# fawnliu/TRIS

Measured on AMD Instinct MI355X. Metric: Stage-1 training images/sec @320px bs48 (TRIS clip-RN50, 3 negatives), higher is better.
Workload: dtype f32 storage/accumulate; products h2 = 2 x f16 pieces; 1 GPU; Stage-1 train step, RefCOCOg-shaped synthetic batch: 48 img/GPU 320x320, 20-token query + 3 negative queries per image, clip-RN50 trunk + frozen aux CLIP ViT-B/32, AdamW (BASELINE.json configs[2]/[3]); per_gpu_batch=48, global_batch=48, size=320, query_len=20, negative_samples=3, parallelism=dp1, sync_bn=False

## Files before the change

### include/tris_hip.h

```cpp
#ifndef TRIS_HIP_H
#define TRIS_HIP_H

#ifdef __cplusplus
extern "C" {
#endif

int tris_gemm_f32(const float* A, const float* B, float* C, int M, int N, int K, long lda, long ldb, long ldc,
                  int transA, int transB, int batch, long strideA, long strideB, long strideC, const float* bias,
                  int bias_mode, const float* resid, long ldr, long strideR, int act, float alpha, float* workspace,
                  long workspace_bytes, void* stream);

int tris_gemm_epilogue_next(float* pre_out, const float* dact_x);

int tris_splitk_tickets_next(int* tickets, int count);
long tris_splitk_fused_launches(void);

int tris_set_gemm_mode(int mode);
int tris_set_gemm_mode_thread(int mode);
int tris_set_option(const char* name, const char* value);
int tris_set_conv_direct_thread(int value);

int tris_set_autotune(int on);
int tris_get_autotune(void);
int tris_get_gemm_mode(void);
// ... 183 lines not shown
int tris_maps_bwd_f32(const float* score, const float* d_relu, const float* d_sig, float* dscore, int B, int h, int w,
                      int N, int S, void* stream);
int tris_resize_bilinear_fwd_f32(const float* X, float* Y, int planes, int Hi, int Wi, int Ho, int Wo,
                                 int align_corners, void* stream);
int tris_resize_bilinear_bwd_f32(const float* dY, float* dX, int planes, int Hi, int Wi, int Ho, int Wo,
                                 int align_corners, void* stream);
int tris_fg_patch_fwd_f32(const float* cam, const float* img, float* patches, int B, int C, int R, int ps,
                          void* stream);
int tris_fg_patch_bwd_f32(const float* dpatches, const float* img, float* dcam, int B, int C, int R, int ps,
                          void* stream);
int tris_vit_assemble_fwd_f32(const float* emb, const float* cls, const float* pos, float* x, int B, int T, int W,
                              void* stream);
int tris_vit_assemble_bwd_f32(const float* dx, float* demb, int B, int T, int W, void* stream);
int tris_stage1_loss_fwd_f32(const float* cls, const float* fi, const float* ft, const float* fneg, int B, int N, int E,
                             int K, float w1, float w4, float w5, float* per_img, float* rowloss, float* losses,
                             void* stream);
int tris_stage1_loss_bwd_f32(const float* cls, const float* fi, const float* ft, const float* fneg, const float* g,
                             float w1, float w4, float w5, int B, int N, int E, int K, float* dcls, float* dfi, void* stream);

int tris_adamw_f32(float* p, const float* g, float* m, float* v, long n, float lr, float beta1, float beta2, float eps,
                   float weight_decay, int step_count, void* stream);
int tris_adamw_dev_f32(float* p, const float* g, float* m, float* v, long n, const float* hyper, float beta1, float beta2,
                       float eps, float weight_decay, void* stream);

int tris_eval_post_f32(const float* relu_map, int S, const unsigned char* target, int oH, int oW, float* cam,
                       long* out_iu, float* workspace , void* stream);

int tris_resample_u8(const unsigned char* in, int Hin, int Win, int C, const int* bounds_h, const int* kk_h, int ksize_h,
                     const int* bounds_v, const int* kk_v, int ksize_v, int Hout, int Wout, unsigned char* tmp,
                     unsigned char* out, void* stream);
int tris_gather2d_u8(const unsigned char* in, int Hin, int Win, int C, const int* yidx, const int* xidx, int Hout,
                     int Wout, unsigned char* out, void* stream);
int tris_mask_sum_nearest_u8(const unsigned char* masks, int K, int Hin, int Win, const int* yidx, const int* xidx,
                             int Hout, int Wout, unsigned char* out, void* stream);
int tris_u8_gather_normalize_f32(const unsigned char* cache, const long* index, int B, long HW, const float* lut,
                                 float* out, int planar, void* stream);
int tris_gather_rows(const void* table, const long* index, long rows, long row_bytes, void* out, void* stream);

#define TRIS_MBOX_MAX_WORLD 16
long tris_mbox_bytes(int cap_floats);
int tris_mbox_alloc(void** ptr, int cap_floats);
int tris_mbox_free(void* ptr);
int tris_mbox_ipc_handle(void* ptr, void* handle64);
int tris_mbox_ipc_open(const void* handle64, void** ptr);
int tris_mbox_ipc_close(void* ptr);
int tris_mbox_exchange_f32(const float* src0, int n0, const float* src1, int n1, float* out, void* const* boxes, int world,
// ... 77 lines not shown
```

### tris_amd/config.py

```python
import contextlib
import os


def _flag(name, default):
    v = os.environ.get(name)
    return default if v is None or v == "" else v != "0"


class _Config:
    def __setattr__(self, name, value):
        if name == "step_graph" and "step_graph" in self.__dict__:
            self.__dict__["step_graph_chosen"] = True
        self.__dict__[name] = value

    def __init__(self):
        e = os.environ.get
        self.step_graph = e("TRIS_STEP_GRAPH", "0")
        self.step_graph_chosen = "TRIS_STEP_GRAPH" in os.environ
        self.hipgraph = _flag("TRIS_HIPGRAPH", True)
        self.text_stream = _flag("TRIS_TEXT_STREAM", True)
        self.wgrad_stream = _flag("TRIS_WGRAD_STREAM", True)
        self.stream_probe = _flag("TRIS_STREAM_PROBE", True)
        self.stream_probe_log = e("TRIS_STREAM_PROBE_LOG") == "1"
        self.text_at = e("TRIS_TEXT_AT", "layer4")
# ... 7 lines not shown
        self.ddp_seg_poison = _flag("TRIS_DDP_SEG_POISON", False)
        self.syncbn_bound = _flag("TRIS_SYNCBN_BOUND", True)
        self.xattn_fused = _flag("TRIS_XATTN_FUSED", True)
        self.xattn_px = _flag("TRIS_XATTN_PX", True)
        self.xattn_h2 = _flag("TRIS_XATTN_H2", True)
        self.xattn_bwd_px = _flag("TRIS_XATTN_BWD_PX", True)
        self.hbm_loader = _flag("TRIS_HBM_LOADER", True)
        self.eval_group = max(1, int(e("TRIS_EVAL_GROUP", "16")))
        self.mbox_spin = int(e("TRIS_MBOX_SPIN", "40000000"))
        self.syncbn_comm = e("TRIS_SYNCBN_COMM", "mailbox")
        self.ddp_check = e("TRIS_DDP_CHECK") == "1"
        self.ddp_sparse_embed = _flag("TRIS_DDP_SPARSE_EMBED", True)
        self.random_init = e("TRIS_RANDOM_INIT") == "1"
        self.h2_planes = _flag("TRIS_H2_PLANES", True)
        self.own_stream = _flag("TRIS_OWN_STREAM", True)
        self.fuse_splitk = _flag("TRIS_FUSE_SPLITK_PY", False)
        self.aux_text_early = _flag("TRIS_AUX_TEXT_EARLY", True)
        self.text_pack = _flag("TRIS_TEXT_PACK", True)
        self.bn_bitmask = _flag("TRIS_BN_BITMASK", True)
        self.gemm_convert = int(e("TRIS_GEMM_CONVERT", "0"))
        self.step_graph_rerecord = int(e("TRIS_STEP_GRAPH_RERECORD", "3"))
        self.side_param_grads = _flag("TRIS_SIDE_PARAM_GRADS", True)
        self.vit_token0 = _flag("TRIS_VIT_TOKEN0", True)

    @contextlib.contextmanager
    def override(self, **kw):
        old = {k: getattr(self, k) for k in kw}
        try:
            for k, v in kw.items():
                setattr(self, k, v)
            yield self
        finally:
            for k, v in old.items():
                setattr(self, k, v)

    def key(self):
        return tuple(sorted((k, v) for k, v in self.__dict__.items() if k not in ("step_graph_chosen", "step_graph_rerecord")))


cfg = _Config()
```

### tris_amd/csrc/optim.hip

```cpp
#include "common.h"
#include "tris_hip.h"

namespace {
__global__ __launch_bounds__(256) void adamw_kernel(float* __restrict__ p, const float* __restrict__ g,
                                                    float* __restrict__ m, float* __restrict__ v, long n, float lr,
                                                    float b1, float b2, float eps, float wd, float bc1, float bc2s) {
  long i = (long)blockIdx.x * blockDim.x + threadIdx.x;
  const long stride = (long)gridDim.x * blockDim.x;
  const long n4 = n >> 2;
  const float decay = 1.0f - lr * wd, step = lr / bc1;
  for (long j = i; j < n4; j += stride) {
    float4 P = *reinterpret_cast<float4*>(p + j * 4), G = *reinterpret_cast<const float4*>(g + j * 4);
    float4 M = *reinterpret_cast<float4*>(m + j * 4), V = *reinterpret_cast<float4*>(v + j * 4);
#define TRIS_ADAM1(e)                       \
  P.e *= decay;                             \
  M.e = b1 * M.e + (1.0f - b1) * G.e;       \
  V.e = b2 * V.e + (1.0f - b2) * G.e * G.e; \
  P.e -= step * M.e / (sqrtf(V.e) / bc2s + eps);
    TRIS_ADAM1(x) TRIS_ADAM1(y) TRIS_ADAM1(z) TRIS_ADAM1(w)
#undef TRIS_ADAM1
    *reinterpret_cast<float4*>(p + j * 4) = P;
    *reinterpret_cast<float4*>(m + j * 4) = M;
    *reinterpret_cast<float4*>(v + j * 4) = V;
  }
  for (long j = n4 * 4 + i; j < n; j += stride) {
    float P = p[j] * decay, G = g[j];
    float M = b1 * m[j] + (1.0f - b1) * G, V = b2 * v[j] + (1.0f - b2) * G * G;
    p[j] = P - step * M / (sqrtf(V) / bc2s + eps);
    m[j] = M;
    v[j] = V;
  }
}
__global__ __launch_bounds__(256) void adamw_dev_kernel(float* __restrict__ p, const float* __restrict__ g,
                                                        float* __restrict__ m, float* __restrict__ v, long n,
                                                        const float* __restrict__ hyper, float b1, float b2, float eps,
                                                        float wd) {
  const float lr = hyper[0], bc1 = hyper[1], bc2s = hyper[2];
  long i = (long)blockIdx.x * blockDim.x + threadIdx.x;
  const long stride = (long)gridDim.x * blockDim.x;
  const long n4 = n >> 2;
  const float decay = 1.0f - lr * wd, step = lr / bc1;
  for (long j = i; j < n4; j += stride) {
    float4 P = *reinterpret_cast<float4*>(p + j * 4), G = *reinterpret_cast<const float4*>(g + j * 4);
    float4 M = *reinterpret_cast<float4*>(m + j * 4), V = *reinterpret_cast<float4*>(v + j * 4);
#define TRIS_ADAM1(e)                       \
  P.e *= decay;                             \
  M.e = b1 * M.e + (1.0f - b1) * G.e;       \
  V.e = b2 * V.e + (1.0f - b2) * G.e * G.e; \
  P.e -= step * M.e / (sqrtf(V.e) / bc2s + eps);
    TRIS_ADAM1(x) TRIS_ADAM1(y) TRIS_ADAM1(z) TRIS_ADAM1(w)
#undef TRIS_ADAM1
    *reinterpret_cast<float4*>(p + j * 4) = P;
    *reinterpret_cast<float4*>(m + j * 4) = M;
    *reinterpret_cast<float4*>(v + j * 4) = V;
  }
  for (long j = n4 * 4 + i; j < n; j += stride) {
    float P = p[j] * decay, G = g[j];
    float M = b1 * m[j] + (1.0f - b1) * G, V = b2 * v[j] + (1.0f - b2) * G * G;
    p[j] = P - step * M / (sqrtf(V) / bc2s + eps);
    m[j] = M;
    v[j] = V;
  }
}
}

extern "C" int tris_adamw_f32(float* p, const float* g, float* m, float* v, long n, float lr, float beta1, float beta2,
                              float eps, float weight_decay, int step_count, void* stream) {
  double bc1 = 1.0 - pow((double)beta1, (double)step_count);
  double bc2 = 1.0 - pow((double)beta2, (double)step_count);
  long g4 = (n / 4 + 255) / 256;
  if (g4 > 8192) g4 = 8192;
  if (g4 < 1) g4 = 1;
  hipLaunchKernelGGL(adamw_kernel, dim3((unsigned)g4), dim3(256), 0, (hipStream_t)stream, p, g, m, v, n, lr, beta1,
                     beta2, eps, weight_decay, (float)bc1, (float)sqrt(bc2));
  TRIS_LAUNCH_CHECK();
  return 0;
}

extern "C" int tris_adamw_dev_f32(float* p, const float* g, float* m, float* v, long n, const float* hyper, float beta1,
                                  float beta2, float eps, float weight_decay, void* stream) {
  long g4 = (n / 4 + 255) / 256;
  if (g4 > 8192) g4 = 8192;
  if (g4 < 1) g4 = 1;
  hipLaunchKernelGGL(adamw_dev_kernel, dim3((unsigned)g4), dim3(256), 0, (hipStream_t)stream, p, g, m, v, n, hyper, beta1,
                     beta2, eps, weight_decay);
  TRIS_LAUNCH_CHECK();
  return 0;
}
```

### tris_amd/graphs.py

```python


import torch


class NotCapturable(RuntimeError):
    """the step cannot be replayed from hipGraphs in this configuration (train_step then runs it eagerly)"""


class GraphedStage1Eval:
    def __init__(self, net, img_shape, query_len, warmup=2):
        assert not net.training, "capture the eval path (model.eval())"
        self.net = net
        dev = next(net.parameters()).device
        self.s_img = torch.zeros(img_shape, device=dev, dtype=torch.float32)
        self.s_ids = torch.zeros(img_shape[0], query_len, device=dev, dtype=torch.int64)
        self.s_ids[:, 0] = 49406
        self.s_ids[:, 1] = 49407
        H = img_shape[2]
        from . import ops
        self.h2_vis, self.h2_txt = ops.h2_private_pool(), ops.h2_private_pool()
        with torch.no_grad():
            side = torch.cuda.Stream()
            side.wait_stream(torch.cuda.current_stream())
            with torch.cuda.stream(side):
# ... 45 lines not shown
        self.s_ids.copy_(ids, non_blocking=True)
        self.g.replay()
        return self.out.clone()


class GraphedTrainStep:

    def __init__(self, model, clip_model, optimizer, args, example, lr_scheduler=None, priming=2):
        from . import ops
        from .CLIP.clip.model import BatchNorm2d
        from .train_stage1 import _step_body
        img, ids, neg = example
        self.model, self.clip_model, self.optimizer, self.args, self.sched = model, clip_model, optimizer, args, lr_scheduler
        self.s_img = img.detach().clone()
        self.s_ids = ids.detach().clone()
        self.s_neg = None if neg is None else neg.detach().clone()
        net = model.module if hasattr(model, "module") else model
        self.bns = [m for m in net.modules() if isinstance(m, BatchNorm2d)]
        optimizer.enable_device_hyper()
        _prime(model, clip_model, optimizer, self.bns, (self.s_img, self.s_ids, self.s_neg), args, priming)
        nbt = [m._nbt_pending for m in self.bns]
        self.g = torch.cuda.CUDAGraph()
        ops._CAPTURE_STREAMS = True
        try:
            with torch.cuda.graph(self.g, capture_error_mode="thread_local"):
                self.losses = _step_body(model, clip_model, optimizer, self.s_img, self.s_ids, self.s_neg, args, None,
                                         device_hyper=True)
        finally:
            ops._CAPTURE_STREAMS = False
        for m, n in zip(self.bns, nbt):
            m._nbt_pending = n

    def __call__(self, img, ids, neg):
        self.s_img.copy_(img, non_blocking=True)
        self.s_ids.copy_(ids, non_blocking=True)
        if self.s_neg is not None:
            self.s_neg.copy_(neg, non_blocking=True)
        opt = self.optimizer
        opt._steps += 1
        opt.push_hyper()
        self.g.replay()
        for m in self.bns:
            m._nbt_pending += 1
        if self.sched is not None:
            self.sched.step()
        return self.losses


def _prime(model, clip_model, optimizer, bns, batch, args, priming, reducer=None):
    from .train_stage1 import _step_body
    keep = [(m.running_mean.clone(), m.running_var.clone(), m._nbt_pending) for m in bns]
    for _ in range(priming):
        _step_body(model, clip_model, optimizer, batch[0], batch[1], batch[2], args, reducer, optimizer_step=False)
    torch.cuda.synchronize()
    with torch.no_grad():
        for m, (rm, rv, nbt) in zip(bns, keep):
            m.running_mean.copy_(rm)
            m.running_var.copy_(rv)
            m._nbt_pending = nbt
    del keep
    torch.cuda.synchronize()
    torch.cuda.empty_cache()


# ... 137 lines not shown
                keys, self.released = self.released, []
                return keys
            g = G()
            _capture(g, self.cap, pool_c, b_heads)
            self.back = [(g,) + wgrad_graphs()[:2] + (take_released(),)]
            self.inline = True
            self.g_btext = G()
            _capture(self.g_btext, self.text, pool_t, lambda: torch.autograd.backward(hidden, h.grad))
            self.inline = False
            self.text_released = take_released()
            n_late = min(6, len(trunk_cuts))
            split = True
            late_sinks = []
            for k, (x, leaf) in enumerate(reversed(trunk_cuts)):
                late = k >= len(trunk_cuts) - n_late
                g = G()
                _capture(g, self.cap, pool_c, lambda: torch.autograd.backward(x, leaf.grad))
                gw, gt, sinks = wgrad_graphs(split=late and split)
                self.back.append((g, gw, gt, take_released()))
                if late:
                    late_sinks += sinks
            self.first_late = len(self.back) - n_late
            spans = self._late_spans(optimizer, late_sinks) if (n_late and self.reducer is None) else None
            self.g_opt_early = None
            if spans:
                early = []
                for gi, a in enumerate(optimizer.arenas):
                    lo, hi = spans.get(gi, (0, 0))
                    early += [(gi, 0, lo), (gi, hi, a.numel)] if hi > lo else [(gi, 0, a.numel)]
                self.g_opt_early = G()
                _capture(self.g_opt_early, self.cap, pool_c, lambda: optimizer.step(device_hyper=True, ranges=early))
                rest = [(gi, lo, hi) for gi, (lo, hi) in spans.items()]
            else:
                rest = None
            self.g_opt_seg, self.g_opt_ranges, self._poisoned, self.poisoned_segments = {}, {}, [], 0
            red = self.reducer
            if red is not None and cfg.ddp_seg_opt and red.segments:
                released = [k for (_, _, _, keys) in self.back for k in keys] + list(self.text_released)
                pool_o = torch.cuda.graph_pool_handle()
                covered = {}
                for k in released:
                    segs = [(ai, s_, e_) for ai, s_, e_ in red.segments.get(k, []) if e_ > s_]
                    if not segs or k in self.g_opt_seg or sorted(red._dense_ranges(k)) != sorted(segs):
                        continue
                    g = G()
                    _capture(g, self.cap, pool_o, lambda: optimizer.step(device_hyper=True, ranges=segs))
                    self.g_opt_seg[k] = g
                    self.g_opt_ranges[k] = segs
                    for ai, s_, e_ in segs:
                        covered.setdefault(ai, []).append((s_, e_))
                if self.g_opt_seg:
                    rest = []
                    for gi, a in enumerate(optimizer.arenas):
                        cur = 0
                        for s_, e_ in sorted(covered.get(gi, [])):
                            if s_ > cur:
                                rest.append((gi, cur, s_))
                            cur = max(cur, e_)
                        if cur < a.numel:
                            rest.append((gi, cur, a.numel))
            self.g_opt = G()
            _capture(self.g_opt, self.cap, pool_c, lambda: optimizer.step(device_hyper=True, ranges=rest))
        finally:
            ops._SEG = None
            ops.h2_end_step()
            self.cuts, self.deferred = [], []
            if gc_was:
                gc.enable()
        del keep, trunk_cuts, h, hidden, vis, late_sinks, fwd
        for m, n in zip(self.bns, nbt):
            m._nbt_pending = n
        self.ev = [torch.cuda.Event() for _ in range(len(self.back) + 8)]
        self.trace = False
        self._marks = None

    def _reduce_and_update(self, red, key):
        from . import ops
        if key in red.done or not red.active:
            return
        n0 = len(red.pending)
        red._launch_now(key)
        g = self.g_opt_seg.get(key)
        if g is not None:
            with torch.cuda.stream(ops.side_stream("reduce")):
                for h in red.pending[n0:]:
# ... 45 lines not shown

    def release(self, key):
        self.released.append(key)

    def defer(self, fn, tensors, sink):
        if self.inline:
            return fn()
        self.deferred.append((fn, tensors, sink))
        return None

    def __call__(self, img, ids, neg):
        from . import ops
        main, text, wg, ev = torch.cuda.current_stream(), self.text, self.wg, self.ev
        tm = self._marks = [] if self.trace else None

        def mark(name, stream=main):
            if tm is not None:
                e = torch.cuda.Event(enable_timing=True)
                e.record(stream)
                tm.append((name, e))
        mark("start")
        if self.h2_pool is not None:
            self.h2_pool.zero_()
            ops.h2_weights_amax(self.h2_arenas)
        self.s_img.copy_(img, non_blocking=True)
        self.s_ids.copy_(ids, non_blocking=True)
        if self.s_neg is not None:
            self.s_neg.copy_(neg, non_blocking=True)
        opt = self.optimizer
        opt._steps += 1
        opt.push_hyper()
        ev[0].record(main)
        fm = self.fwd_marks
        from .config import cfg as _cfg
        aux_early = bool(_cfg.aux_text_early)
        for i, g in enumerate(self.fwd):
            if i == fm.get("text", 0):
                if i:
                    ev[0].record(main)
                text.wait_event(ev[0])
                with torch.cuda.stream(text):
                    self.g_ftext.replay()
                    ev[1].record(text)
                    mark("text_fwd_done", text)
                    if aux_early:
                        self.g_faux.replay()
                        ev[7 + len(self.back)].record(text)
# ... 41 lines not shown
            if gt is not None:
                text.wait_event(e)
                with torch.cuda.stream(text):
                    gt.replay()
                    mark(f"w{i}t_done", text)
            if red is not None:
                for k in keys:
                    self._reduce_and_update(red, k)
            if i == self.first_late - 1:
                ev[4].record(wg)
        if self.g_opt_early is not None:
            main.wait_event(ev[4])
            main.wait_event(ev[2])
            self.g_opt_early.replay()
            mark("opt_early_done")
        ev[3].record(wg)
        ev[5].record(text)
        main.wait_event(ev[3])
        main.wait_event(ev[5])
        mark("joined")
        if red is not None:
            red.finish()
        self.g_opt.replay()
        if self._poisoned:
            for v, saved in self._poisoned:
                v.copy_(saved)
                saved.record_stream(main)
            self._poisoned = []
        mark("opt_done")
        for m in self.bns:
            m._nbt_pending += 1
        if self.sched is not None:
            self.sched.step()
        return self.losses


def frozen_text(clip_model, ids):
    from . import ops
    from .config import cfg
    if not cfg.hipgraph or torch.cuda.is_current_stream_capturing() or torch.is_grad_enabled():
        return clip_model.encode_text_hidden(ids)
    n, L = ids.shape
    cache = clip_model.__dict__.setdefault("_tris_text_graphs", {})
    key = (n, L, clip_model.token_embedding.weight.data_ptr(), ops.get_gemm_mode(), cfg.text_pack)
    g = cache.get(key)
    if g is None:
# ... 5 lines not shown
```

### tris_amd/ops.py

```python
import math
import os

import torch

from . import _lib
from ._lib import CONSTS, call, query
from .config import cfg

EW = CONSTS


class NoGpuError(RuntimeError):
    pass


_RAW_STREAM = getattr(torch._C, "_cuda_getCurrentRawStream", None)


def _stream():
    if _RAW_STREAM is not None:
        return _RAW_STREAM(torch.cuda.current_device())
    return torch.cuda.current_stream().cuda_stream


# ... 461 lines not shown
    return True


class GradBox:
    __slots__ = ("value", "consumed")

    def __init__(self):
        self.value = None
        self.consumed = False

    def deposit(self, g):
        if self.consumed or self.value is not None:
            return False
        self.value = g
        return True


_H2 = {"pool": None, "next": 0, "step": 0, "paused": 0, "arenas": [], "const": None, "const_next": 0, "const_tags": {}}
_H2_STEP_IDS = [0]
H2_SLOTS = 4096
H2_SUB = 2048
H2_CONST_SLOTS = 1024
H2_PREPASS_MAX = 1 << 25
H2_AUTO_KEEP = 4


def h2_on():
    return _ARITH == "h2" and not _H2["paused"] and not _thread_mode_is_set()


_H2_ARENAS = []


def h2_register_arena(arena):
    import weakref
    r = weakref.ref(arena)
    _H2_ARENAS.append(r)
    for p in arena.params:
        p._tris_arena = r


def _h2_live_arenas():
    out, words = [], 0
    for r in reversed(list(_H2_ARENAS)):
        a = r()
        if a is None or not a.params or getattr(a.params[0], "_tris_arena", None) is not r:
            _H2_ARENAS.remove(r)
        elif _H2["pool"] is not None and a.p.device == _H2["pool"].device and words + len(a.params) <= H2_SLOTS // 2:
            out.append(a)
            words += len(a.params)
    return out


def h2_weights_amax(arenas=None):
    base = 0
    for a in (_h2_live_arenas() if arenas is None else arenas):
        if not hasattr(a, "_h2_dev"):
            a._h2_dev = (torch.tensor(list(a.offsets), device=a.p.device, dtype=torch.int64),
                         torch.tensor([p.numel() for p in a.params], device=a.p.device, dtype=torch.int64))
        call("tris_amax_segments_f32", P(a.p), a._h2_dev[0].data_ptr(), a._h2_dev[1].data_ptr(), len(a.params),
             _H2["pool"].data_ptr() + 4 * H2_SUB * base, _stream())
        if cfg.h2_planes:
            if not hasattr(a, "_pl_dev"):
                idx = [i for i, p in enumerate(a.params) if _pl_weight_ok(p)]
                a._pl_idx = idx
                a._pl_dev = None if not idx else (
                    torch.tensor([a.offsets[i] for i in idx], device=a.p.device, dtype=torch.int64),
                    torch.tensor([a.params[i].numel() for i in idx], device=a.p.device, dtype=torch.int64),
                    torch.tensor(idx, device=a.p.device, dtype=torch.int64))
                a.pl = torch.zeros_like(a.p) if idx else None
            if a._pl_dev is not None:
                call("tris_h2_planes_segments_f32", P(a.p), a._pl_dev[0].data_ptr(), a._pl_dev[1].data_ptr(), a._pl_dev[2].data_ptr(),
                     len(a._pl_idx), _H2["pool"].data_ptr() + 4 * H2_SUB * base, P(a.pl), _stream())
            if not hasattr(a, "_plt_dev"):
                idt = [i for i in getattr(a, "_pl_idx", []) if _pl_weight_t_ok(a.params[i])]
                a._plt_idx = idt
                mk = lambda v: torch.tensor(v, device=a.p.device, dtype=torch.int64)
                a._plt_dev = None if not idt else (mk([a.offsets[i] for i in idt]), mk([a.params[i].shape[0] for i in idt]),
                                                   mk([a.params[i].shape[1] for i in idt]), mk(idt))
                a.plt = torch.zeros_like(a.p) if idt else None
            if a._plt_dev is not None:
                call("tris_h2_planes_t_segments_f32", P(a.p), a._plt_dev[0].data_ptr(), a._plt_dev[1].data_ptr(), a._plt_dev[2].data_ptr(),
                     a._plt_dev[3].data_ptr(), len(a._plt_idx), _H2["pool"].data_ptr() + 4 * H2_SUB * base, P(a.plt), _stream())
        base += len(a.params)
    return base


def _pl_weight_t_ok(p):
    if p.dim() == 2:
        return cfg.gemm_convert > 0 and getattr(p, "_tris_linear_w", False) and p.shape[0] % 64 == 0 and p.shape[1] % 64 == 0
    return p.dim() == 4 and p.shape[2] * p.shape[3] == 1 and p.shape[0] % 64 == 0 and p.shape[1] % 64 == 0


def _pl_weight_ok(p):
    if p.dim() == 2:
        return cfg.gemm_convert > 0 and getattr(p, "_tris_linear_w", False) and p.shape[1] % 8 == 0 and p.is_contiguous()
    return p.dim() == 4 and p.shape[1] % 8 == 0 and (p.is_contiguous(memory_format=torch.channels_last) or p.shape[2] * p.shape[3] == 1)


def _a_planes(A, M, K):
    slot = _h2_amax(A)
    if slot is None:
        return A
    t = torch.empty_like(A)
    call("tris_h2_planes_f32", P(A), P(t), A.numel(), slot, _stream())
    PL_STATS["converted"] = PL_STATS.get("converted", 0) + 1
    return pl_tag(t, slot)

# ... 9 lines not shown
    _H2["in_step"] = bool(explicit)
    wgrad_join()
    dev = torch.device("cuda", torch.cuda.current_device())
    live = _H2.setdefault("auto_pools", {})
    if _H2["pool"] is None or _H2["pool"].device != dev:
        _H2["pool"] = torch.zeros(H2_SLOTS * H2_SUB, device=dev, dtype=torch.int32)
        live.clear()
    elif not explicit and _H2.get("auto_grad") and not _H2.get("private") and not torch.cuda.is_current_stream_capturing():
        live[_H2["step"]] = _H2["pool"]
        while len(live) > H2_AUTO_KEEP:
            live.pop(next(iter(live)))
        _H2["pool"] = torch.zeros(H2_SLOTS * H2_SUB, device=dev, dtype=torch.int32)
    else:
        if explicit:
            live.clear()
        _H2["pool"].zero_()
    _H2["auto_grad"] = (not explicit) and torch.is_grad_enabled() and not _H2.get("private")
    _H2["step"] = _h2_new_step_id()
    _H2["plane_numel"] = {}
    _PL_GRAD.clear()
    base = 0
    arenas = _h2_live_arenas() if not _H2.get("private") else []
    for a in arenas:
        for i, p in enumerate(a.params):
            p._h2 = (_H2["step"], _H2["pool"].data_ptr() + 4 * H2_SUB * (base + i), p._version)
        base += len(a.params)
    _H2["next"] = _H2["base"] = base
    _H2["arenas"] = arenas
    h2_weights_amax(arenas)
    if cfg.h2_planes:
        for a in arenas:
            for i in (a._pl_idx if getattr(a, "pl", None) is not None else ()):
                p = a.params[i]
                p._plw = (_H2["step"], a.pl.data_ptr() + 4 * a.offsets[i], p._h2[1])
                _H2["plane_numel"][p._h2[1]] = p.numel()
            for i in (a._plt_idx if getattr(a, "plt", None) is not None else ()):
                p = a.params[i]
                p._plwt = (_H2["step"], a.plt.data_ptr() + 4 * a.offsets[i], p._h2[1])
    return _H2["pool"]


def h2_end_step():
    _H2["in_step"] = False


def h2_auto_step():
    if not planes_on() or _H2.get("in_step") or _H2.get("auto_lock") or _H2.get("private"):
        return False
    if _H2["pool"] is not None and _H2["next"] == _H2.get("base", -1):
        return False
    h2_begin_step(explicit=False)
    return True
# ... 102 lines not shown
        return None
    import weakref
    slot = _H2["const"].data_ptr() + 4 * H2_SUB * _H2["const_next"]
    _H2["const_next"] += 1
    call("tris_amax_bits_f32", P(t), t.numel(), slot, _stream())
    _H2["const_tags"][key] = (t._version, t.data_ptr(), slot, weakref.ref(t))
    return slot


def _h2_amax(t):
    slot = _h2_tag_slot(t)
    if slot is not None:
        return slot
    dense = t.is_contiguous() or (t.dim() == 4 and t.is_contiguous(memory_format=torch.channels_last))
    if not (t.numel() <= H2_PREPASS_MAX and dense and t.data_ptr() % 16 == 0 and t.numel() > 0):
        return None
    if isinstance(t, torch.nn.Parameter) and not getattr(t, "_tris_arena", False):
        slot = _h2_const_slot(t)
        if slot is not None:
            return slot
    slot = _h2_slot()
    if slot is None:
        return None
    call("tris_amax_bits_f32", P(t), t.numel(), slot, _stream())
    try:
        t._h2 = (_H2["step"], slot, t._version)
    except AttributeError:
        pass
    return slot


def h2_arm(A, B, a_slot=None, b_slot=None):
    if not h2_on():
        return False
    a = a_slot if a_slot is not None else (_h2_amax(A) if A is not None else None)
    b = None
    if a is not None:
        b = b_slot if b_slot is not None else (_h2_amax(B) if B is not None else None)
    if a is None or b is None:
        return False
    call("tris_h2_next", a, b, 0.0, 0.0)
    return True


PL_STATS = {"unplanes": 0, "dx_planes": 0, "dy_planes": 0, "products": 0, "mixed": 0, "last": False, "last_t": False}

# ... 10 lines not shown

def pl_word(t):
    tag = getattr(t, "_pl", None) if t is not None else None
    if tag is None:
        return None
    if (tag[0] != _H2["step"] and tag[0] not in _H2.get("auto_pools", ())) or tag[2] != t.data_ptr():
        raise RuntimeError("a plane tensor outlived the step whose amax pool scales it")
    return tag[1]


def pl_tag(t, word):
    t._pl = (_H2["step"], word, t.data_ptr())
    t._h2 = (_H2["step"], word, t._version)
    _H2.setdefault("plane_numel", {})[word] = t.numel()
    return t


def h2_range_report(threshold=0.01):
    numel = _H2.get("plane_numel") or {}
    pool = _H2["pool"]
    if pool is None or not numel:
        return {"plane_tensors": 0, "elements": 0, "elements_below_floor": 0, "max_fraction_below_floor": 0.0, "out_of_range_operands": 0}
    torch.cuda.synchronize()
    base = pool.data_ptr()
    words = sorted(numel)
    idx = torch.tensor([(w - base) // (4 * H2_SUB) for w in words], device=pool.device, dtype=torch.int64)
    cnt = pool.view(-1, H2_SUB)[idx][:, 1::16].to(torch.int64).sum(1).cpu().tolist()
    fr = [c / max(numel[w], 1) for c, w in zip(cnt, words)]
    return {"plane_tensors": len(words), "elements": int(sum(numel.values())), "elements_below_floor": int(sum(cnt)),
            "max_fraction_below_floor": max(fr), "out_of_range_operands": sum(1 for f in fr if f > threshold)}


def _unplanes_raw(t, cache=True):
    w = pl_word(t)
    c = getattr(t, "_pl_f32", None) if cache else None
    if c is None:
        c = torch.empty_like(t)
        call("tris_h2_unplanes_f32", P(t), P(c), t.numel(), w, _stream())
        c._h2 = (_H2["step"], w, c._version)
        if cache:
            t._pl_f32 = c
        PL_STATS["unplanes"] += 1
    return c


class _UnplanesFn(torch.autograd.Function):

    @staticmethod
    def forward(ctx, t):
        return _unplanes_raw(t, cache=False)
# ... 2201 lines not shown
```

### tris_amd/optim.py

```python
import torch

from . import _lib, ops

ALIGN = 64


class Arena:
    def __init__(self, params):
        self.params = [p for p in params if p.requires_grad and not getattr(p, "_tris_no_grad_path", False)]
        dev = self.params[0].device
        offs, n = [], 0
        for p in self.params:
            offs.append(n)
            n += (p.numel() + ALIGN - 1) // ALIGN * ALIGN
        self.numel = n
        self.p = torch.zeros(n, device=dev, dtype=torch.float32)
        self.g = torch.zeros(n, device=dev, dtype=torch.float32)
        self.m = torch.zeros(n, device=dev, dtype=torch.float32)
        self.v = torch.zeros(n, device=dev, dtype=torch.float32)
        self.offsets = offs
        for p, o in zip(self.params, offs):
            pv, gv = self._view(self.p, p, o), self._view(self.g, p, o)
            with torch.no_grad():
                pv.copy_(p.data)
# ... 56 lines not shown
        ev = torch.cuda.Event()
        ev.record()
        self._ring_ev[slot] = ev

    def zero_grad(self, set_to_none=False):
        for a in self.arenas:
            for p in a.params:
                if p._tris_accumulates:
                    p.grad.zero_()
        return None

    def span(self, params):
        want = {id(p) for p in params if getattr(p, "_tris_sink", False)}
        for gi, a in enumerate(self.arenas):
            idx = [i for i, p in enumerate(a.params) if id(p) in want]
            if not idx:
                continue
            if len(idx) != len(want) or idx != list(range(idx[0], idx[-1] + 1)):
                return None
            hi = a.offsets[idx[-1] + 1] if idx[-1] + 1 < len(a.params) else a.numel
            return gi, a.offsets[idx[0]], hi
        return None

    @torch.no_grad()
    def step(self, closure=None, device_hyper=False, ranges=None):
        ops.wgrad_join()
        st = torch.cuda.current_stream().cuda_stream
        if device_hyper:
            hy = self.enable_device_hyper()
            if ranges is None:
                ranges = [(gi, 0, a.numel) for gi, a in enumerate(self.arenas)]
            for gi, lo, hi in ranges:
                if hi <= lo:
                    continue
                g, a = self.param_groups[gi], self.arenas[gi]
                b1, b2 = g["betas"]
                o = lo * 4
                _lib.call("tris_adamw_dev_f32", a.p.data_ptr() + o, a.g.data_ptr() + o, a.m.data_ptr() + o, a.v.data_ptr() + o,
                          hi - lo, hy[gi].data_ptr(), float(b1), float(b2), float(g["eps"]), float(g["weight_decay"]), st)
            return
        assert ranges is None
        self._steps += 1
        for g, a in zip(self.param_groups, self.arenas):
            b1, b2 = g["betas"]
            _lib.call("tris_adamw_f32", a.p.data_ptr(), a.g.data_ptr(), a.m.data_ptr(), a.v.data_ptr(), a.numel,
                      float(g["lr"]), float(b1), float(b2), float(g["eps"]), float(g["weight_decay"]), self._steps, st)

    def _index(self):
        out, base = [], 0
        for gi, (g, a) in enumerate(zip(self.param_groups, self.arenas)):
            out.append((gi, g, a, {id(p): o for p, o in zip(a.params, a.offsets)}, base))
            base += len(g["params"])
        return out

    def state_dict(self):
        state, groups = {}, []
        for gi, g, a, offs, base in self._index():
            if self._steps > 0:
                for j, p in enumerate(g["params"]):
                    o = offs.get(id(p))
                    if o is None:
                        continue
                    state[base + j] = {"step": torch.tensor(float(self._steps)),
                                       "exp_avg": Arena._view(a.m, p, o).detach().clone(),
                                       "exp_avg_sq": Arena._view(a.v, p, o).detach().clone()}
            pg = {k: v for k, v in g.items() if k != "params"}
            pg["params"] = list(range(base, base + len(g["params"])))
            groups.append(pg)
        return {"state": state, "param_groups": groups}
# ... 34 lines not shown
```

### tris_amd/train_stage1.py

```python
import datetime
import logging
import os
import random
import time

import numpy as np
import torch

from . import ops
from .config import cfg
from .loss.clip_loss import clip_forward

CLIP_INPUT = 224


def MaxLoss(x):
    return -(torch.log(x.clamp(0.0001, 0.9999))).mean()


def stage1_forward_losses(model, clip_model, img, word_ids, neg_word_ids, args):
    B = img.shape[0]
    from .graphs import frozen_text
    from .model.model_stage1 import _overlap_enabled, _side_stream
    f_all = None
# ... 31 lines not shown
    vit = clip_model.visual
    f_i = vit.forward_patches(ops.fg_patches(cam, im, vit.patch_size))
    with torch.no_grad():
        if f_all is None:
            f_all = clip_model.encode_text_hidden(ids_all)
        elif callable(f_all):
            f_all = f_all()
        f_t = f_all[:B].contiguous()
        f_neg = f_all[B:].reshape(B, K, -1).contiguous() if K > 0 else None
    return ops.stage1_loss(cls, f_i, f_t, f_neg, float(args.w1), float(args.w4), float(args.w5))


def _step_body(model, clip_model, optimizer, img, word_ids, neg_word_ids, args, reducer, device_hyper=False,
               optimizer_step=True):
    ops.h2_begin_step()
    losses, _, _ = stage1_forward_losses(model, clip_model, img, word_ids, neg_word_ids, args)
    optimizer.zero_grad()
    if reducer is not None:
        reducer.begin_step()
    losses[0].backward()
    if reducer is not None:
        reducer.reduce()
    if optimizer_step:
        optimizer.step(device_hyper=device_hyper)
    else:
        ops.wgrad_join()
    ops.h2_end_step()
    return losses.detach()


def _graphable(model, optimizer, img, reducer):
    if cfg.step_graph not in ("1", "seg") or ops._PROF is not None:
        return False
    if not img.is_cuda or not hasattr(optimizer, "enable_device_hyper") or torch.cuda.is_current_stream_capturing():
        return False
    from .CLIP.clip.model import BatchNorm2d
    net = model.module if hasattr(model, "module") else model
    if not net.training:
        return False
    sync_bn = any(m.process_group is not None for m in net.modules() if isinstance(m, BatchNorm2d))
    if cfg.step_graph == "1":
        return reducer is None and not sync_bn
    if sync_bn:
        from . import comm
        if any(m is None for m in comm.Mailbox._by_group.values()) or cfg.syncbn_comm != "mailbox":
            return False
    return True
# ... 261 lines not shown
```

Baseline: 1371 img/s.

## Fuse weight amax and h2 plane build into AdamW step, carry to next step

```diff
diff --git a/include/tris_hip.h b/include/tris_hip.h
--- a/include/tris_hip.h
+++ b/include/tris_hip.h
@@ -229,6 +229,12 @@
                    float weight_decay, int step_count, void* stream);
 int tris_adamw_dev_f32(float* p, const float* g, float* m, float* v, long n, const float* hyper, float beta1, float beta2,
                        float eps, float weight_decay, void* stream);
+int tris_adamw_amax_f32(float* p, const float* g, float* m, float* v, long n, float lr, float beta1, float beta2, float eps,
+                        float weight_decay, int step_count, long lo, const long* seg_offs, int nseg, unsigned* words,
+                        void* stream);
+int tris_adamw_dev_amax_f32(float* p, const float* g, float* m, float* v, long n, const float* hyper, float beta1, float beta2,
+                            float eps, float weight_decay, long lo, const long* seg_offs, int nseg, unsigned* words,
+                            void* stream);
 
 int tris_eval_post_f32(const float* relu_map, int S, const unsigned char* target, int oH, int oW, float* cam,
                        long* out_iu, float* workspace , void* stream);
diff --git a/tris_amd/config.py b/tris_amd/config.py
--- a/tris_amd/config.py
+++ b/tris_amd/config.py
@@ -53,6 +53,7 @@
         self.step_graph_rerecord = int(e("TRIS_STEP_GRAPH_RERECORD", "3"))
         self.side_param_grads = _flag("TRIS_SIDE_PARAM_GRADS", True)
         self.vit_token0 = _flag("TRIS_VIT_TOKEN0", True)
+        self.adamw_planes = _flag("TRIS_ADAMW_PLANES", True)
 
     @contextlib.contextmanager
     def override(self, **kw):
diff --git a/tris_amd/csrc/optim.hip b/tris_amd/csrc/optim.hip
--- a/tris_amd/csrc/optim.hip
+++ b/tris_amd/csrc/optim.hip
@@ -1,10 +1,23 @@
 #include "common.h"
 #include "tris_hip.h"
+#include "optim_plan.h"
 
 namespace {
-__global__ __launch_bounds__(256) void adamw_kernel(float* __restrict__ p, const float* __restrict__ g,
-                                                    float* __restrict__ m, float* __restrict__ v, long n, float lr,
-                                                    float b1, float b2, float eps, float wd, float bc1, float bc2s) {
+#include "amax.h"
+
+__device__ __forceinline__ void adam4(float4& P, const float4 G, float4& M, float4& V, float decay, float step, float b1, float b2,
+                                      float eps, float bc2s) {
+#define TRIS_ADAM1(e)                       \
+  P.e *= decay;                             \
+  M.e = b1 * M.e + (1.0f - b1) * G.e;       \
+  V.e = b2 * V.e + (1.0f - b2) * G.e * G.e; \
+  P.e -= step * M.e / (sqrtf(V.e) / bc2s + eps);
+  TRIS_ADAM1(x) TRIS_ADAM1(y) TRIS_ADAM1(z) TRIS_ADAM1(w)
+#undef TRIS_ADAM1
+}
+__device__ __forceinline__ void adam_range(float* __restrict__ p, const float* __restrict__ g, float* __restrict__ m,
+                                           float* __restrict__ v, long n, float lr, float b1, float b2, float eps, float wd,
+                                           float bc1, float bc2s) {
   long i = (long)blockIdx.x * blockDim.x + threadIdx.x;
   const long stride = (long)gridDim.x * blockDim.x;
   const long n4 = n >> 2;
@@ -12,13 +25,7 @@
   for (long j = i; j < n4; j += stride) {
     float4 P = *reinterpret_cast<float4*>(p + j * 4), G = *reinterpret_cast<const float4*>(g + j * 4);
     float4 M = *reinterpret_cast<float4*>(m + j * 4), V = *reinterpret_cast<float4*>(v + j * 4);
-#define TRIS_ADAM1(e)                       \
-  P.e *= decay;                             \
-  M.e = b1 * M.e + (1.0f - b1) * G.e;       \
-  V.e = b2 * V.e + (1.0f - b2) * G.e * G.e; \
-  P.e -= step * M.e / (sqrtf(V.e) / bc2s + eps);
-    TRIS_ADAM1(x) TRIS_ADAM1(y) TRIS_ADAM1(z) TRIS_ADAM1(w)
-#undef TRIS_ADAM1
+    adam4(P, G, M, V, decay, step, b1, b2, eps, bc2s);
     *reinterpret_cast<float4*>(p + j * 4) = P;
     *reinterpret_cast<float4*>(m + j * 4) = M;
     *reinterpret_cast<float4*>(v + j * 4) = V;
@@ -31,36 +38,80 @@
     v[j] = V;
   }
 }
+__global__ __launch_bounds__(256) void adamw_kernel(float* __restrict__ p, const float* __restrict__ g,
+                                                    float* __restrict__ m, float* __restrict__ v, long n, float lr,
+                                                    float b1, float b2, float eps, float wd, float bc1, float bc2s) {
+  adam_range(p, g, m, v, n, lr, b1, b2, eps, wd, bc1, bc2s);
+}
 __global__ __launch_bounds__(256) void adamw_dev_kernel(float* __restrict__ p, const float* __restrict__ g,
                                                         float* __restrict__ m, float* __restrict__ v, long n,
                                                         const float* __restrict__ hyper, float b1, float b2, float eps,
                                                         float wd) {
-  const float lr = hyper[0], bc1 = hyper[1], bc2s = hyper[2];
-  long i = (long)blockIdx.x * blockDim.x + threadIdx.x;
-  const long stride = (long)gridDim.x * blockDim.x;
-  const long n4 = n >> 2;
+  adam_range(p, g, m, v, n, hyper[0], b1, b2, eps, wd, hyper[1], hyper[2]);
+}
+
+__device__ __forceinline__ void amax_flush(int seg, unsigned mx, unsigned* __restrict__ words) {
+  bool pend = mx != 0u;
+  while (__any(pend)) {
+    const int leader = __ffsll((unsigned long long)__ballot(pend)) - 1;
+    const int s0 = __shfl(seg, leader, 64);
+    amax_commit((pend && seg == s0) ? mx : 0u, words + (long)s0 * 2048);
+    if (seg == s0) pend = false;
+  }
+}
+template <bool DEV>
+__global__ __launch_bounds__(256) void adamw_amax_kernel(float* __restrict__ p, const float* __restrict__ g,
+                                                         float* __restrict__ m, float* __restrict__ v, long n4, long piece4,
+                                                         long lo, const long* __restrict__ seg_offs, int nseg,
+                                                         unsigned* __restrict__ words, const float* __restrict__ hyper, float lr,
+                                                         float bc1, float bc2s, float b1, float b2, float eps, float wd) {
+  if (DEV) {
+    lr = hyper[0];
+    bc1 = hyper[1];
+    bc2s = hyper[2];
+  }
   const float decay = 1.0f - lr * wd, step = lr / bc1;
-  for (long j = i; j < n4; j += stride) {
-    float4 P = *reinterpret_cast<float4*>(p + j * 4), G = *reinterpret_cast<const float4*>(g + j * 4);
-    float4 M = *reinterpret_cast<float4*>(m + j * 4), V = *reinterpret_cast<float4*>(v + j * 4);
-#define TRIS_ADAM1(e)                       \
-  P.e *= decay;                             \
-  M.e = b1 * M.e + (1.0f - b1) * G.e;       \
-  V.e = b2 * V.e + (1.0f - b2) * G.e * G.e; \
-  P.e -= step * M.e / (sqrtf(V.e) / bc2s + eps);
-    TRIS_ADAM1(x) TRIS_ADAM1(y) TRIS_ADAM1(z) TRIS_ADAM1(w)
-#undef TRIS_ADAM1
-    *reinterpret_cast<float4*>(p + j * 4) = P;
-    *reinterpret_cast<float4*>(m + j * 4) = M;
-    *reinterpret_cast<float4*>(v + j * 4) = V;
+  const long beg = (long)blockIdx.x * piece4;
+  const long end = beg + piece4 < n4 ? beg + piece4 : n4;
+  int seg = -1;
+  unsigned mx = 0u;
+  for (long j0 = beg; j0 < end; j0 += 256) {
+    const long j = j0 + threadIdx.x;
+    const bool act = j < end;
+    int s = seg;
+    unsigned a = 0u;
+    if (act) {
+      float4 P = *reinterpret_cast<float4*>(p + j * 4), G = *reinterpret_cast<const float4*>(g + j * 4);
+      float4 M = *reinterpret_cast<float4*>(m + j * 4), V = *reinterpret_cast<float4*>(v + j * 4);
+      adam4(P, G, M, V, decay, step, b1, b2, eps, bc2s);
+      *reinterpret_cast<float4*>(p + j * 4) = P;
+      *reinterpret_cast<float4*>(m + j * 4) = M;
+      *reinterpret_cast<float4*>(v + j * 4) = V;
+      a = abits4(P);
+      const long pos = lo + j * 4;
+      if (s < 0) {
+        int l = 0, h = nseg - 1;
+        while (l < h) {
+          const int mid = (l + h + 1) >> 1;
+          if (seg_offs[mid] <= pos) l = mid; else h = mid - 1;
+        }
+        s = l;
+      } else {
+        while (s + 1 < nseg && seg_offs[s + 1] <= pos) ++s;
+      }
+    }
+    if (__any(act && seg >= 0 && s != seg)) {
+      amax_flush(seg, mx, words);
+      mx = 0u;
+    }
+    seg = s;
+    mx = max(mx, a);
   }
-  for (long j = n4 * 4 + i; j < n; j += stride) {
-    float P = p[j] * decay, G = g[j];
-    float M = b1 * m[j] + (1.0f - b1) * G, V = b2 * v[j] + (1.0f - b2) * G * G;
-    p[j] = P - step * M / (sqrtf(V) / bc2s + eps);
-    m[j] = M;
-    v[j] = V;
-  }
+  amax_flush(seg, mx, words);
+}
+
+inline bool amax_args_ok(long n, long lo, const long* seg_offs, int nseg, const unsigned* words) {
+  return n > 0 && (n & 63) == 0 && lo >= 0 && (lo & 63) == 0 && seg_offs != nullptr && nseg >= 1 && words != nullptr;
 }
 }
 
@@ -87,3 +138,32 @@
   TRIS_LAUNCH_CHECK();
   return 0;
 }
+
+extern "C" int tris_adamw_amax_f32(float* p, const float* g, float* m, float* v, long n, float lr, float beta1, float beta2,
+                                   float eps, float weight_decay, int step_count, long lo, const long* seg_offs, int nseg,
+                                   unsigned* words, void* stream) {
+  if (!amax_args_ok(n, lo, seg_offs, nseg, words)) return (int)hipErrorInvalidValue;
+  double bc1 = 1.0 - pow((double)beta1, (double)step_count);
+  double bc2 = 1.0 - pow((double)beta2, (double)step_count);
+  unsigned grid;
+  long piece4;
+  tris_adamw_plan(n >> 2, &grid, &piece4);
+  hipLaunchKernelGGL(adamw_amax_kernel<false>, dim3(grid), dim3(256), 0, (hipStream_t)stream, p, g, m, v, n >> 2, piece4, lo,
+                     seg_offs, nseg, words, (const float*)nullptr, lr, (float)bc1, (float)sqrt(bc2), beta1, beta2, eps,
+                     weight_decay);
+  TRIS_LAUNCH_CHECK();
+  return 0;
+}
+
+extern "C" int tris_adamw_dev_amax_f32(float* p, const float* g, float* m, float* v, long n, const float* hyper, float beta1,
+                                       float beta2, float eps, float weight_decay, long lo, const long* seg_offs, int nseg,
+                                       unsigned* words, void* stream) {
+  if (!amax_args_ok(n, lo, seg_offs, nseg, words) || hyper == nullptr) return (int)hipErrorInvalidValue;
+  unsigned grid;
+  long piece4;
+  tris_adamw_plan(n >> 2, &grid, &piece4);
+  hipLaunchKernelGGL(adamw_amax_kernel<true>, dim3(grid), dim3(256), 0, (hipStream_t)stream, p, g, m, v, n >> 2, piece4, lo,
+                     seg_offs, nseg, words, hyper, 0.0f, 1.0f, 1.0f, beta1, beta2, eps, weight_decay);
+  TRIS_LAUNCH_CHECK();
+  return 0;
+}
diff --git a/tris_amd/csrc/optim_plan.h b/tris_amd/csrc/optim_plan.h
--- /dev/null
+++ b/tris_amd/csrc/optim_plan.h
@@ -0,0 +1,11 @@
+#pragma once
+
+inline void tris_adamw_plan(long n4, unsigned* grid, long* piece4) {
+  if (n4 < 1) n4 = 1;
+  long blocks = (n4 + 255) / 256;
+  if (blocks > 8192) blocks = 8192;
+  long piece = (n4 + blocks - 1) / blocks;
+  piece = (piece + 255) / 256 * 256;
+  *piece4 = piece;
+  *grid = (unsigned)((n4 + piece - 1) / piece);
+}
diff --git a/tris_amd/graphs.py b/tris_amd/graphs.py
--- a/tris_amd/graphs.py
+++ b/tris_amd/graphs.py
@@ -91,12 +91,17 @@
         nbt = [m._nbt_pending for m in self.bns]
         self.g = torch.cuda.CUDAGraph()
         ops._CAPTURE_STREAMS = True
+        ops._H2["defer_weights"] = []
+        if hasattr(optimizer, "prepare_carry"):
+            optimizer.prepare_carry()
         try:
             with torch.cuda.graph(self.g, capture_error_mode="thread_local"):
                 self.losses = _step_body(model, clip_model, optimizer, self.s_img, self.s_ids, self.s_neg, args, None,
                                          device_hyper=True)
         finally:
             ops._CAPTURE_STREAMS = False
+            self.h2_deferred = ops._H2.pop("defer_weights")
+        self.carry = bool(self.h2_deferred) and bool(getattr(optimizer, "last_carried", False))
         for m, n in zip(self.bns, nbt):
             m._nbt_pending = n
 
@@ -106,9 +111,14 @@
         if self.s_neg is not None:
             self.s_neg.copy_(neg, non_blocking=True)
         opt = self.optimizer
+        if self.h2_deferred:
+            from . import ops
+            ops.h2_weights_ready(self.h2_deferred)
         opt._steps += 1
         opt.push_hyper()
         self.g.replay()
+        if self.carry:
+            opt.carried()
         for m in self.bns:
             m._nbt_pending += 1
         if self.sched is not None:
@@ -292,6 +302,7 @@
                     late_sinks += sinks
             self.first_late = len(self.back) - n_late
             spans = self._late_spans(optimizer, late_sinks) if (n_late and self.reducer is None) else None
+            carried = []
             self.g_opt_early = None
             if spans:
                 early = []
@@ -299,7 +310,8 @@
                     lo, hi = spans.get(gi, (0, 0))
                     early += [(gi, 0, lo), (gi, hi, a.numel)] if hi > lo else [(gi, 0, a.numel)]
                 self.g_opt_early = G()
-                _capture(self.g_opt_early, self.cap, pool_c, lambda: optimizer.step(device_hyper=True, ranges=early))
+                optimizer.prepare_carry(early)
+                carried.append(_capture(self.g_opt_early, self.cap, pool_c, lambda: optimizer.step(device_hyper=True, ranges=early)))
                 rest = [(gi, lo, hi) for gi, (lo, hi) in spans.items()]
             else:
                 rest = None
@@ -314,7 +326,7 @@
                     if not segs or k in self.g_opt_seg or sorted(red._dense_ranges(k)) != sorted(segs):
                         continue
                     g = G()
-                    _capture(g, self.cap, pool_o, lambda: optimizer.step(device_hyper=True, ranges=segs))
+                    _capture(g, self.cap, pool_o, lambda: optimizer.step(device_hyper=True, ranges=segs, carry=False))
                     self.g_opt_seg[k] = g
                     self.g_opt_ranges[k] = segs
                     for ai, s_, e_ in segs:
@@ -330,7 +342,11 @@
                         if cur < a.numel:
                             rest.append((gi, cur, a.numel))
             self.g_opt = G()
-            _capture(self.g_opt, self.cap, pool_c, lambda: optimizer.step(device_hyper=True, ranges=rest))
+            if self.reducer is None:
+                optimizer.prepare_carry(rest)
+            carried.append(_capture(self.g_opt, self.cap, pool_c,
+                                    lambda: optimizer.step(device_hyper=True, ranges=rest, carry=self.reducer is None)))
+            self.carry = all(carried)
         finally:
             ops._SEG = None
             ops.h2_end_step()
@@ -422,7 +438,7 @@
         mark("start")
         if self.h2_pool is not None:
             self.h2_pool.zero_()
-            ops.h2_weights_amax(self.h2_arenas)
+            ops.h2_weights_ready(self.h2_arenas)
         self.s_img.copy_(img, non_blocking=True)
         self.s_ids.copy_(ids, non_blocking=True)
         if self.s_neg is not None:
@@ -510,6 +526,8 @@
         if red is not None:
             red.finish()
         self.g_opt.replay()
+        if self.carry:
+            opt.carried()
         if self._poisoned:
             for v, saved in self._poisoned:
                 v.copy_(saved)
diff --git a/tris_amd/ops.py b/tris_amd/ops.py
--- a/tris_amd/ops.py
+++ b/tris_amd/ops.py
@@ -507,6 +507,7 @@
 H2_SUB = 2048
 H2_CONST_SLOTS = 1024
 H2_PREPASS_MAX = 1 << 25
+H2_PREPASS_LOG = None
 H2_AUTO_KEEP = 4
 
 
@@ -537,38 +538,90 @@
     return out
 
 
+def _h2_arena_setup(a):
+    if hasattr(a, "h2w"):
+        return
+    mk = lambda v: torch.tensor(v, device=a.p.device, dtype=torch.int64)
+    a._h2_dev = (mk(list(a.offsets)), mk([p.numel() for p in a.params]))
+    a._h2_ends = mk(list(a.offsets) + [a.numel])
+    a._pl_idx = [i for i, p in enumerate(a.params) if _pl_weight_ok(p)]
+    a._plt_idx = [i for i in a._pl_idx if _pl_weight_t_ok(a.params[i])]
+    a.pl = a.plt = None
+    a._pl_tabs = {}
+    a.h2w = torch.zeros(len(a.params) * H2_SUB, device=a.p.device, dtype=torch.int32)
+
+
+def h2_plane_tables(a, seg_ranges=None):
+    _h2_arena_setup(a)
+    key = None if seg_ranges is None else tuple(seg_ranges)
+    tabs = a._pl_tabs.get(key)
+    if tabs is None:
+        inside = lambda i: key is None or any(s0 <= i < s1 for s0, s1 in key)
+        mk = lambda v: torch.tensor(v, device=a.p.device, dtype=torch.int64)
+        idx = [i for i in a._pl_idx if inside(i)]
+        idt = [i for i in a._plt_idx if inside(i)]
+        tabs = a._pl_tabs[key] = (
+            None if not idx else (mk([a.offsets[i] for i in idx]), mk([a.params[i].numel() for i in idx]), mk(idx)),
+            None if not idt else (mk([a.offsets[i] for i in idt]), mk([a.params[i].shape[0] for i in idt]),
+                                  mk([a.params[i].shape[1] for i in idt]), mk(idt)))
+    return tabs
+
+
+def h2_weight_planes(a, seg_ranges=None):
+    pl, plt = h2_plane_tables(a, seg_ranges)
+    if a.pl is None and a._pl_idx:
+        a.pl = torch.zeros_like(a.p)
+    if a.plt is None and a._plt_idx:
+        a.plt = torch.zeros_like(a.p)
+    if pl is not None:
+        call("tris_h2_planes_segments_f32", P(a.p), pl[0].data_ptr(), pl[1].data_ptr(), pl[2].data_ptr(), len(pl[2]),
+             a.h2w.data_ptr(), P(a.pl), _stream())
+    if plt is not None:
+        call("tris_h2_planes_t_segments_f32", P(a.p), plt[0].data_ptr(), plt[1].data_ptr(), plt[2].data_ptr(), plt[3].data_ptr(),
+             len(plt[3]), a.h2w.data_ptr(), P(a.plt), _stream())
+
+
 def h2_weights_amax(arenas=None):
-    base = 0
     for a in (_h2_live_arenas() if arenas is None else arenas):
-        if not hasattr(a, "_h2_dev"):
-            a._h2_dev = (torch.tensor(list(a.offsets), device=a.p.device, dtype=torch.int64),
-                         torch.tensor([p.numel() for p in a.params], device=a.p.device, dtype=torch.int64))
+        _h2_arena_setup(a)
+        a._carry = None
+        a.h2w.zero_()
         call("tris_amax_segments_f32", P(a.p), a._h2_dev[0].data_ptr(), a._h2_dev[1].data_ptr(), len(a.params),
-             _H2["pool"].data_ptr() + 4 * H2_SUB * base, _stream())
+             a.h2w.data_ptr(), _stream())
         if cfg.h2_planes:
-            if not hasattr(a, "_pl_dev"):
-                idx = [i for i, p in enumerate(a.params) if _pl_weight_ok(p)]
-                a._pl_idx = idx
-                a._pl_dev = None if not idx else (
-                    torch.tensor([a.offsets[i] for i in idx], device=a.p.device, dtype=torch.int64),
-                    torch.tensor([a.params[i].numel() for i in idx], device=a.p.device, dtype=torch.int64),
-                    torch.tensor(idx, device=a.p.device, dtype=torch.int64))
-                a.pl = torch.zeros_like(a.p) if idx else None
-            if a._pl_dev is not None:
-                call("tris_h2_planes_segments_f32", P(a.p), a._pl_dev[0].data_ptr(), a._pl_dev[1].data_ptr(), a._pl_dev[2].data_ptr(),
-                     len(a._pl_idx), _H2["pool"].data_ptr() + 4 * H2_SUB * base, P(a.pl), _stream())
-            if not hasattr(a, "_plt_dev"):
-                idt = [i for i in getattr(a, "_pl_idx", []) if _pl_weight_t_ok(a.params[i])]
-                a._plt_idx = idt
-                mk = lambda v: torch.tensor(v, device=a.p.device, dtype=torch.int64)
-                a._plt_dev = None if not idt else (mk([a.offsets[i] for i in idt]), mk([a.params[i].shape[0] for i in idt]),
-                                                   mk([a.params[i].shape[1] for i in idt]), mk(idt))
-                a.plt = torch.zeros_like(a.p) if idt else None
-            if a._plt_dev is not None:
-                call("tris_h2_planes_t_segments_f32", P(a.p), a._plt_dev[0].data_ptr(), a._plt_dev[1].data_ptr(), a._plt_dev[2].data_ptr(),
-                     a._plt_dev[3].data_ptr(), len(a._plt_idx), _H2["pool"].data_ptr() + 4 * H2_SUB * base, P(a.plt), _stream())
-        base += len(a.params)
-    return base
+            h2_weight_planes(a)
+
+
+def _h2_carry_print(a):
+    return a.p._version, sum(p._version for p in a.params)
+
+
+def h2_carry_wanted(a):
+    return bool(cfg.adamw_planes and planes_on() and hasattr(a, "h2w") and any(a is b for b in _H2.get("arenas", ())))
+
+
+def h2_carry_set(a, optimizer):
+    import weakref
+    a._carry = (weakref.ref(optimizer), optimizer._steps, _h2_carry_print(a))
+
+
+def _h2_carry_valid(a):
+    c = getattr(a, "_carry", None)
+    if c is None or not cfg.adamw_planes or not cfg.h2_planes or not hasattr(a, "h2w"):
+        return False
+    opt = c[0]()
+    return opt is not None and opt._steps == c[1] and c[2] == _h2_carry_print(a)
+
+
+def h2_weights_ready(arenas):
+    n = 0
+    capturing = torch.cuda.is_current_stream_capturing()
+    for a in arenas:
+        if not capturing and _h2_carry_valid(a):
+            n += 1
+        else:
+            h2_weights_amax([a])
+    return n
 
 
 def _pl_weight_t_ok(p):
@@ -624,12 +677,16 @@
     base = 0
     arenas = _h2_live_arenas() if not _H2.get("private") else []
     for a in arenas:
+        _h2_arena_setup(a)
         for i, p in enumerate(a.params):
-            p._h2 = (_H2["step"], _H2["pool"].data_ptr() + 4 * H2_SUB * (base + i), p._version)
+            p._h2 = (_H2["step"], a.h2w.data_ptr() + 4 * H2_SUB * i, p._version)
         base += len(a.params)
     _H2["next"] = _H2["base"] = base
     _H2["arenas"] = arenas
-    h2_weights_amax(arenas)
+    if _H2.get("defer_weights") is not None and cfg.adamw_planes and planes_on() and torch.cuda.is_current_stream_capturing():
+        _H2["defer_weights"] += arenas
+    else:
+        h2_weights_ready(arenas)
     if cfg.h2_planes:
         for a in arenas:
             for i in (a._pl_idx if getattr(a, "pl", None) is not None else ()):
@@ -778,6 +835,13 @@
     slot = _h2_slot()
     if slot is None:
         return None
+    if H2_PREPASS_LOG is not None:
+        import sys
+        f = sys._getframe(1)
+        while f.f_back is not None and f.f_code.co_name in ("h2_arm", "h2_pp", "_a_planes", "_pl_weight"):
+            f = f.f_back
+        key = (f"{f.f_code.co_name}:{f.f_lineno}", tuple(t.shape))
+        H2_PREPASS_LOG[key] = H2_PREPASS_LOG.get(key, 0) + 1
     call("tris_amax_bits_f32", P(t), t.numel(), slot, _stream())
     try:
         t._h2 = (_H2["step"], slot, t._version)
@@ -834,10 +898,16 @@
     if pool is None or not numel:
         return {"plane_tensors": 0, "elements": 0, "elements_below_floor": 0, "max_fraction_below_floor": 0.0, "out_of_range_operands": 0}
     torch.cuda.synchronize()
-    base = pool.data_ptr()
     words = sorted(numel)
-    idx = torch.tensor([(w - base) // (4 * H2_SUB) for w in words], device=pool.device, dtype=torch.int64)
-    cnt = pool.view(-1, H2_SUB)[idx][:, 1::16].to(torch.int64).sum(1).cpu().tolist()
+    cnt = [0] * len(words)
+    for buf in [pool] + [a.h2w for a in _H2.get("arenas", ()) if hasattr(a, "h2w")]:
+        base, n = buf.data_ptr(), buf.numel() // H2_SUB
+        sel = [(k, (w - base) // (4 * H2_SUB)) for k, w in enumerate(words) if base <= w < base + 4 * H2_SUB * n]
+        if not sel:
+            continue
+        idx = torch.tensor([i for _, i in sel], device=buf.device, dtype=torch.int64)
+        for (k, _), c in zip(sel, buf.view(-1, H2_SUB)[idx][:, 1::16].to(torch.int64).sum(1).cpu().tolist()):
+            cnt[k] = c
     fr = [c / max(numel[w], 1) for c, w in zip(cnt, words)]
     return {"plane_tensors": len(words), "elements": int(sum(numel.values())), "elements_below_floor": int(sum(cnt)),
             "max_fraction_below_floor": max(fr), "out_of_range_operands": sum(1 for f in fr if f > threshold)}
diff --git a/tris_amd/optim.py b/tris_amd/optim.py
--- a/tris_amd/optim.py
+++ b/tris_amd/optim.py
@@ -102,29 +102,73 @@
             return gi, a.offsets[idx[0]], hi
         return None
 
+    def _seg_ranges(self, a, parts):
+        first = getattr(a, "_seg_first", None)
+        if first is None:
+            first = a._seg_first = {o: i for i, o in enumerate(a.offsets)}
+            first[a.numel] = len(a.offsets)
+        out = [(first.get(lo), first.get(hi)) for lo, hi in parts]
+        return None if any(s0 is None or s1 is None for s0, s1 in out) else out
+
+    def prepare_carry(self, ranges=None):
+        for gi, a in enumerate(self.arenas):
+            parts = [(0, a.numel)] if ranges is None else [(lo, hi) for g, lo, hi in ranges if g == gi and hi > lo]
+            segs = self._seg_ranges(a, parts) if (parts and hasattr(a, "h2w")) else None
+            if segs:
+                ops.h2_plane_tables(a, None if parts == [(0, a.numel)] else segs)
+
+    def carried(self):
+        for a in self.arenas:
+            ops.h2_carry_set(a, self)
+
     @torch.no_grad()
-    def step(self, closure=None, device_hyper=False, ranges=None):
+    def step(self, closure=None, device_hyper=False, ranges=None, carry=True):
         ops.wgrad_join()
         st = torch.cuda.current_stream().cuda_stream
+        capturing = torch.cuda.is_current_stream_capturing()
+        full = ranges is None
         if device_hyper:
             hy = self.enable_device_hyper()
-            if ranges is None:
-                ranges = [(gi, 0, a.numel) for gi, a in enumerate(self.arenas)]
-            for gi, lo, hi in ranges:
-                if hi <= lo:
-                    continue
-                g, a = self.param_groups[gi], self.arenas[gi]
-                b1, b2 = g["betas"]
-                o = lo * 4
-                _lib.call("tris_adamw_dev_f32", a.p.data_ptr() + o, a.g.data_ptr() + o, a.m.data_ptr() + o, a.v.data_ptr() + o,
-                          hi - lo, hy[gi].data_ptr(), float(b1), float(b2), float(g["eps"]), float(g["weight_decay"]), st)
-            return
-        assert ranges is None
-        self._steps += 1
-        for g, a in zip(self.param_groups, self.arenas):
+        else:
+            assert ranges is None
+            self._steps += 1
+        if ranges is None:
+            ranges = [(gi, 0, a.numel) for gi, a in enumerate(self.arenas)]
+        all_carried = bool(carry)
+        for gi, a in enumerate(self.arenas):
+            parts = [(lo, hi) for g_, lo, hi in ranges if g_ == gi and hi > lo]
+            if not parts:
+                continue
+            g = self.param_groups[gi]
             b1, b2 = g["betas"]
-            _lib.call("tris_adamw_f32", a.p.data_ptr(), a.g.data_ptr(), a.m.data_ptr(), a.v.data_ptr(), a.numel,
-                      float(g["lr"]), float(b1), float(b2), float(g["eps"]), float(g["weight_decay"]), self._steps, st)
+            tail = (float(b1), float(b2), float(g["eps"]), float(g["weight_decay"]))
+            segs = self._seg_ranges(a, parts) if (carry and ops.h2_carry_wanted(a)) else None
+            key = None if parts == [(0, a.numel)] else (tuple(segs) if segs else None)
+            if segs and capturing and key not in a._pl_tabs:
+                segs = None
+            if not segs:
+                all_carried = False
+                a._carry = None
+            for k, (lo, hi) in enumerate(parts):
+                ptrs = tuple(t.data_ptr() + 4 * lo for t in (a.p, a.g, a.m, a.v))
+                if segs:
+                    s0, s1 = segs[k]
+                    a.h2w[s0 * ops.H2_SUB:s1 * ops.H2_SUB].zero_()
+                    more = (lo, a._h2_ends.data_ptr(), len(a.params), a.h2w.data_ptr(), st)
+                    if device_hyper:
+                        _lib.call("tris_adamw_dev_amax_f32", *ptrs, hi - lo, hy[gi].data_ptr(), *tail, *more)
+                    else:
+                        _lib.call("tris_adamw_amax_f32", *ptrs, hi - lo, float(g["lr"]), *tail, self._steps, *more)
+                elif device_hyper:
+                    _lib.call("tris_adamw_dev_f32", *ptrs, hi - lo, hy[gi].data_ptr(), *tail, st)
+                else:
+                    _lib.call("tris_adamw_f32", *ptrs, hi - lo, float(g["lr"]), *tail, self._steps, st)
+            if segs:
+                ops.h2_weight_planes(a, key and list(key))
+        if all_carried and full and not capturing:
+            self.carried()
+        self.last_carried = all_carried
+        return all_carried
 
     def _index(self):
         out, base = [], 0
diff --git a/tris_amd/train_stage1.py b/tris_amd/train_stage1.py
--- a/tris_amd/train_stage1.py
+++ b/tris_amd/train_stage1.py
@@ -77,7 +77,7 @@
     if reducer is not None:
         reducer.reduce()
     if optimizer_step:
-        optimizer.step(device_hyper=device_hyper)
+        optimizer.step(device_hyper=device_hyper, **({"carry": False} if reducer is not None else {}))
     else:
         ops.wgrad_join()
     ops.h2_end_step()
```

After: 1378 img/s (median of 6 runs). About the same (+0.5%).
